# sloisel/MultiGridBarrier.jl

Measured on AMD Instinct MI355X. Metric: Newton iters/sec + wall-clock to converge, 2D P2 p-Laplace L=9, higher is better.
Workload: dtype f64

## Files before the change

multigridbarrier.jl_amd/csrc/api.cpp:

```cpp
#include <chrono>
#include <cmath>
#include <cstring>
#include <algorithm>
#include <limits>
#include <memory>
#include <string>

#include "closest.hpp"
#include "contour.hpp"
#include "faces.hpp"
#include "figure.hpp"
#include "interpolate.hpp"
#include "polyline.hpp"
#include "problem.hpp"
#include "quadrature.hpp"
#include "raycast.hpp"
#include "stream.hpp"
#include "surface.hpp"
#include "tubes.hpp"
#include "weld.hpp"

using namespace mgbhip;

mgbhip_problem* problem_create(mgbhip_ctx* ctx, const mgbhip_problem_desc* d, mgbhip_problem* share);
// ... 327 lines not shown
}

int mgbhip_set_hessian(mgbhip_problem* P, int32_t level, const double* values) {
    MGB_API_BEGIN_ON(P)
    check_level(P, level);
    MGB_REQUIRE(values, "null argument");
    P->ensure_plan(level);
    mgbhip::Level& L = P->levels[level];
    MGB_REQUIRE(L.Hval.n >= (size_t)L.nnz, "this level keeps no CSR value array");
    L.Hval.upload(values, (size_t)L.nnz, P->stream());
    MGB_HIP_CHECK(hipStreamSynchronize(P->stream()));
    L.H.set_from_outside();
    return MGBHIP_OK;
    MGB_API_END
}

int mgbhip_solve_newton(mgbhip_problem* P, int32_t level, const double* g, double* x, double* lambda2) {
    MGB_API_BEGIN_ON(P)
    check_level(P, level);
    MGB_REQUIRE(g && x, "null argument");
    hipStream_t st = P->stream();
    const size_t m = (size_t)P->levels[level].m;
    P->d_g.upload(g, m, st);
    P->factor(level, P->d_g.p);
    P->trisolve_carried(level, P->d_nv.p);
    int status = P->levels[level].solver.status(st);
    if (status != MGBHIP_OK && P->lu_fallback(level, P->d_g.p, P->d_nv.p)) status = MGBHIP_OK;
    P->d_nv.download(x, m, st);
    MGB_HIP_CHECK(hipStreamSynchronize(st));
    if (lambda2) {
        double acc = 0.0;
        for (size_t i = 0; i < m; ++i) acc += g[i] * x[i];
        *lambda2 = acc;
    }
    if (status != MGBHIP_OK) g_last_error = "Cholesky met a non-positive pivot";
    return status;
    MGB_API_END
}

int mgbhip_problem_set_sharding(mgbhip_problem* P, int32_t level, int64_t n_iface, const int32_t* iface_cols, const double* own_mask) {
    MGB_API_BEGIN_ON(P)
    check_level(P, level);
    mgbhip::Level& L = P->levels[level];
    MGB_REQUIRE(!L.solver.analyzed, "sharding must be set before the first solve of the level");
    MGB_REQUIRE(own_mask != nullptr && n_iface >= 0 && n_iface <= L.m && (n_iface == 0 || iface_cols), "bad sharding arguments");
    L.h_iface.assign(iface_cols, iface_cols + n_iface);
    for (int64_t i = 0; i < n_iface; ++i) {
// ... 8 lines not shown
    MGB_API_END
}

int mgbhip_problem_set_collective(mgbhip_problem* P, mgbhip_allreduce_fn fn, void* user, int32_t accepts_device_ptr) {
    MGB_API_BEGIN_ON(P)
    P->coll_fn = fn;
    P->coll_user = user;
    P->coll_device = accepts_device_ptr != 0;
    return MGBHIP_OK;
    MGB_API_END
}

int mgbhip_newton_direction(mgbhip_problem* P, int32_t level, const double* s, const double* c, const double* z0, double* x,
                            double* lambda2, int32_t* condensed) {
    MGB_API_BEGIN_ON(P)
    check_level(P, level);
    MGB_REQUIRE(s && c && z0 && x, "null argument");
    hipStream_t st = P->stream();
    const size_t m = (size_t)P->levels[level].m;
    stage_inputs(P, level, s, c, z0);
    P->eval_f1(level, P->d_x.p, P->d_z0.p, P->d_c.p, P->d_g.p);
    P->eval_f2(level, P->d_x.p, P->d_z0.p, P->d_c.p, false, P->d_g.p);
    if (condensed) *condensed = P->levels[level].H.condensed() ? 1 : 0;
    P->factor(level, P->d_g.p);
    P->trisolve_carried(level, P->d_nv.p);
    const int status = P->levels[level].solver.status(st);
    P->d_nv.download(x, m, st);
    if (lambda2) {
        std::vector<double> g(m);
        P->d_g.download(g.data(), m, st);
        MGB_HIP_CHECK(hipStreamSynchronize(st));
        double acc = 0.0;
        for (size_t i = 0; i < m; ++i) acc += g[i] * x[i];
        *lambda2 = acc;
    }
    MGB_HIP_CHECK(hipStreamSynchronize(st));
    if (status != MGBHIP_OK) g_last_error = "Cholesky met a non-positive pivot";
    return status;
    MGB_API_END
}

int mgbhip_trial_values(mgbhip_problem* P, int32_t level, const double* x, const double* dir, double step, const double* c,
                        const double* z0, double* y, double* g, double* xn, int32_t* moved, int32_t* finite, int32_t* path) {
    MGB_API_BEGIN_ON(P)
    check_level(P, level);
    MGB_REQUIRE(x && dir && c && z0 && y && g && xn && moved && finite && path, "null argument");
    MGB_REQUIRE(!P->sharded(), "trial_values: not for sharded problems");
// ... 1283 lines not shown
```

multigridbarrier.jl_amd/csrc/driver.cpp:

```cpp
#include <chrono>
#include <cstdio>
#include <cstdlib>
#include <cmath>
#include <cstring>
#include <functional>
#include <limits>

#include "problem.hpp"

using namespace mgbhip;

namespace {

constexpr double EPS = std::numeric_limits<double>::epsilon();

bool debug_on() {
    static const bool on = env_on("MGBHIP_DEBUG");
    return on;
}
#define DBG(...) do { if (debug_on()) { fprintf(stderr, __VA_ARGS__); } } while (0)

struct Stop {
    double lambda_tol;
    double theta;
// ... 172 lines not shown
        if (P->sharded()) { P->d_gpart.ensure((size_t)C.m); P->d_gnpart.ensure((size_t)C.m); }
        C.F1(P->d_x.p, P->d_g.p, P->d_gpart.p);
        gs = vec_stats(P, C.level, P->d_g.p, C.m);
    }
    double ymin = y;
    if (gs.bad != 0.0 || !std::isfinite(gs.sumsq)) throw InvalidArgument("newton: initial gradient has non-finite entries");
    double gnorm = std::sqrt(gs.sumsq);
    double gmin = gnorm;
    double incmin = INFINITY;
    int k = 0;
    bool converged = false;
    Level& L = P->levels[C.level];
    struct RobustReset {
        MfSolver& s;
        ~RobustReset() { s.robust = false; }
    } robust_reset{L.solver};
    while (k < maxit && !converged) {
        ++k;
        C.F2(P->d_x.p);
        auto t0 = std::chrono::steady_clock::now();
        int fstatus = MGBHIP_OK;
        int leaf_flag = 0;
        for (int attempt = 0; attempt < 2; ++attempt) {
            P->factor(C.level, C.rhs_of_g());
            P->trisolve_carried(C.level, P->d_nv.p);
            const double seq = P->next_seq();
            launch_dir_finish(P->d_nv.p, P->d_g.p, C.m, P->d_scratch.p, P->d_scal.p, L.solver.status_flags_rw(), P->pin.dev, st,
                              P->own_mask(C.level), seq);
            L.solver.flags_cleared();
            P->wait_results(seq);
            P->pin.i[1] = P->pin.d[5] != 0.0 ? 1 : 0;
            leaf_flag |= P->pin.d[6] != 0.0 ? 1 : 0;
            P->pin.i[2] = leaf_flag;
            fstatus = MfSolver::status_from(P->pin.i + 1, L.solver.factored_condensed);
            if (P->sharded()) {
                P->pin.d[5] = fstatus != MGBHIP_OK ? 1.0 : 0.0;
                P->allreduce_host(P->pin.d + 2, 4, 0);
                fstatus = P->pin.d[5] != 0.0 ? MGBHIP_ERR_NOT_SPD : MGBHIP_OK;
            }
            const bool at_floor = std::fabs(P->pin.d[4]) <= EPS * std::fmax(std::fabs(y), 1.0);
            const bool suspicious = fstatus != MGBHIP_OK || P->pin.d[3] != 0.0 || !std::isfinite(P->pin.d[2]) ||
                                    (!(P->pin.d[4] > 0) && !at_floor);
            if (!suspicious || attempt == 1 || !L.solver.has_inverse_path() || L.solver.robust) break;
            DBG("newton[lev %d] k=%d: direction rejected (status %d, lambda^2=%.3e): refactoring with the substitution kernels\n",
                C.level, k, fstatus, P->pin.d[4]);
            L.solver.robust = true;
            L.H.drop_factors();
// ... 288 lines not shown
```

multigridbarrier.jl_amd/csrc/kernels.hpp:

```cpp
#pragma once
#include "common.hpp"
#include "cone.hpp"
#include "elem_layout.hpp"
#include "panel_layout.hpp"

namespace mgbhip {

struct LeafDesc {
    int64_t F_off;
    int32_t interior;
    uint32_t packed;
};

struct ElemParams {
    int32_t p, nu, nD, nstage;
    int32_t ymask;
    int64_t N, n;
    const double* ops[MGBHIP_MAX_OPS];
    const double* stage_ptr[MGBHIP_MAX_OPS];
    int32_t D_state[MGBHIP_MAX_ND];
    int32_t D_op[MGBHIP_MAX_ND];
    int32_t D_stage[MGBHIP_MAX_ND];
    const double* w;
    const double* c;
// ... 60 lines not shown
void launch_restrict_trial(int64_t rows, const int32_t* ptr, const int32_t* col, const double* val, const double* ret, double* g,
                            double* scratch, const double* x, const double* nn, double s, double* xn, int32_t* moved, int32_t stamp,
                            hipStream_t st);
void launch_publish(const double* src, int n, double* host_block, int host_lo, double seq, hipStream_t st);
void launch_dir_finish(const double* v, const double* g, int64_t n, double* scratch, double* scal, int32_t* status2, double* host,
                       hipStream_t st, const double* mask = nullptr, double seq = 0.0);
void launch_trial_finish(const double* g, int64_t n, double* scratch, const double* f0_partials, int64_t f0_count, double* scal,
                         int32_t* moved, double* host, hipStream_t st, const double* mask = nullptr, double seq = 0.0,
                         bool partials_ready = false);
void launch_index_gather(const double* v, const int32_t* idx, int64_t cnt, double* out, hipStream_t st);
void launch_index_scatter(const double* in, const int32_t* idx, int64_t cnt, double* v, hipStream_t st);
int64_t reduce_scratch_doubles(int64_t n);

void launch_csr_matvec(int64_t rows, const int32_t* ptr, const int32_t* col, const double* val,
                       const double* x, double* y, bool add, bool long_rows, hipStream_t st);
int csr_chunks(int64_t max_row_len);
void launch_csr_matvec_chunked(int64_t rows, const int32_t* ptr, const int32_t* col, const double* val,
                               const double* x, double* y, double* scratch, int nchunk, hipStream_t st);
void launch_prolong(int64_t rows, const int32_t* ptr, const int32_t* col, const double* val, const double* s,
                    const double* z0, double* zfull, hipStream_t st);
void launch_step(const double* x, const double* n, double s, double* xn, int64_t len, int32_t* moved, int32_t stamp,
                 hipStream_t st);
void launch_scale_copy(const double* src, double alpha, double* dst, int64_t len, hipStream_t st);
void launch_border_tail(const double* g, double* tail, int64_t m, hipStream_t st);
void launch_axpy(double alpha, const double* x, double* y, int64_t len, hipStream_t st);
void launch_fill(double value, double* y, int64_t len, hipStream_t st);

void launch_gather_shared(int64_t nshared, const int32_t* sh_q, const int32_t* cptr, const int32_t* cidx, const double* slab,
                          double* out, hipStream_t st);
void launch_gather_assemble(int64_t nnz, const int32_t* cptr, const int32_t* cidx, const double* slab,
                            double* Hval, bool long_lists, hipStream_t st, int32_t chunk = 0, int32_t nchunk = 0,
                            double* part = nullptr, const int32_t* qmap = nullptr, int64_t nq = 0);

struct PanelParams {
    int32_t p, nu;
    int64_t N;
    const int32_t* ecol_ptr;
    const double* panels;
    const int32_t* eoff;
    const double* hel;
    double* slab;
    int32_t cmax;
    int32_t upper_only;
    const int32_t* spos;
};
bool launch_panel_project_mfma(const PanelParams& P, hipStream_t st);
void launch_invert_lists(const int32_t* cidx, int64_t total, int32_t* spos, hipStream_t st);
// ... 7 lines not shown
```

multigridbarrier.jl_amd/csrc/mf_launch_plan.hpp:

```cpp
#pragma once
#include <algorithm>
#include <cstdint>
#include <cstdlib>
#include <vector>

#include "host_util.hpp"
#include "mf_analysis.hpp"

namespace mgbhip {

struct MfLaunch {
    int32_t first, count;
    int32_t cls;
    int32_t max_m, max_k;
    int32_t max_child = 0;
    bool tiny = false;
    bool wave = false;
    bool inv = false;
    bool iface = false;
    int32_t grec_first = -1;
};

constexpr int BIG_INV_MAX_M = 7000;
constexpr int GATHER_MAX_CHILD = 8;
constexpr int BIG_DIAG0_MIN_COUNT = 24;

struct MfSwitches {
    bool no_geo;
    bool old_big;
    bool merge_groups;
    bool packed_leaves;
    bool wave_small;
    int64_t inv_min_n;
    int64_t wave_min_n;
    bool gather_lds_maps;
    int gather_ct;
    bool bwd_split;
    static MfSwitches from_env() {
        auto num = [](const char* name, long long dflt) { const char* e = getenv(name); return e ? atoll(e) : dflt; };
        return {env_on("MGBHIP_NO_GEO"), env_on("MGBHIP_OLD_BIG"), !env_on("MGBHIP_NO_MERGE_GROUPS"), !env_on("MGBHIP_NO_PACKED_LEAVES"),
                !env_on("MGBHIP_NO_WAVE_SMALL"), num("MGBHIP_INV_MIN_N", 1024), num("MGBHIP_WAVE_MIN_N", 0),
                env_on("MGBHIP_GATHER_LDS_MAPS"), (int)num("MGBHIP_GATHER_CT", 0), num("MGBHIP_BWD_SPLIT", 1) != 0};
    }
};

using LevelLaunches = std::vector<std::vector<MfLaunch>>;

inline MfLaunch launch_of_range(const MfPlan& plan, MfLaunch L, int32_t first, int32_t count) {
    L.first = first; L.count = count;
    L.max_m = 0; L.max_k = 0; L.max_child = 0;
    for (int32_t t = first; t < first + count; ++t) {
        L.max_m = std::max(L.max_m, plan.fronts[t].m);
        L.max_k = std::max(L.max_k, plan.fronts[t].k);
        L.max_child = std::max(L.max_child, plan.fronts[t].nchild);
    }
    return L;
}

inline void merge_straggler_groups(const MfPlan& plan, std::vector<MfLaunch>& G) {
    auto absorb = [&](size_t into, size_t from) {
        MfLaunch& A = G[into];
        const MfLaunch& B = G[from];
        A.first = B.first;
        A.count += B.count;
        A.max_k = std::max(A.max_k, B.max_k);
// ... 118 lines not shown
                    if (par >= 0 && on_big_path[par]) return false;
                    any = true;
                }
    return any;
}

enum MfAssembly : int32_t { MF_ASM_NONE = 0, MF_ASM_GATHER = 1, MF_ASM_COLS = 2 };
enum MfBlock0 : int32_t { MF_B0_NA = 0, MF_B0_GATHER = 1, MF_B0_DIAG0 = 2, MF_B0_STEP0 = 3 };
enum MfBackward : int32_t { MF_BWD_NA = 0, MF_BWD_K8 = 1, MF_BWD_K16 = 2, MF_BWD_GENERAL = 3 };

inline size_t big_gather_lds(const MfLaunch& L) { return (size_t)L.max_child * (size_t)L.max_m * sizeof(int32_t); }
inline MfAssembly big_assembly_kind(const MfLaunch& L) {
    if (L.cls) return MF_ASM_NONE;
    if (L.max_child < 1 || L.max_child > GATHER_MAX_CHILD || big_gather_lds(L) > 40 * 1024) return MF_ASM_COLS;
    return MF_ASM_GATHER;
}
inline MfBlock0 big_block0_kind(const MfLaunch& L, bool inv) {
    if (L.cls || !inv) return MF_B0_NA;
    if (!L.iface && big_assembly_kind(L) == MF_ASM_GATHER) return MF_B0_GATHER;
    return (L.iface || L.count >= BIG_DIAG0_MIN_COUNT) ? MF_B0_DIAG0 : MF_B0_STEP0;
}
inline int backward_small_kmax(const MfLaunch& L) { return L.max_k <= 8 ? 8 : (L.max_k <= 16 ? 16 : 0); }

constexpr int GATHER_MIN_WGS = 768;
inline int big_gather_ct(const MfLaunch& L, int forced) {
    if (forced == 8 || forced == 16 || forced == 32) return forced;
    int ct = 8;
    while (ct < 32 && (int64_t)L.count * ((L.max_m + 2 * ct - 1) / (2 * ct)) >= GATHER_MIN_WGS) ct *= 2;
    return ct;
}

constexpr int BWD_SPLIT_MAX = 16;
constexpr int BWD_SPLIT_CUS = 256;
constexpr int BWD_SPLIT_COLS = 64;
constexpr int BWD_THIN_BOUNDARY = 8;
inline int bwd_inv_split(int32_t count, int32_t max_k, int32_t max_m) {
    if (count < 1 || max_m - max_k <= BWD_THIN_BOUNDARY) return 1;
    return std::max(1, std::min({BWD_SPLIT_MAX, BWD_SPLIT_CUS / count, (max_k + BWD_SPLIT_COLS - 1) / BWD_SPLIT_COLS}));
}
inline int32_t bwd_split_stride(int32_t max_k) { return (max_k + 1) & ~1; }
inline void bwd_split_scratch(const LevelLaunches& solves, int64_t out[2]) {
    out[0] = out[1] = 0;
    for (auto& lev : solves)
        for (auto& L : lev) {
            if (L.count == 0 || L.cls || !L.inv || bwd_inv_split(L.count, L.max_k, L.max_m) == 1) continue;
            out[0] = std::max<int64_t>(out[0], L.count);
// ... 61 lines not shown
```

multigridbarrier.jl_amd/csrc/mf_numeric.hip:

```cpp
#include <hip/hip_runtime.h>

#include <cstdio>

#include <algorithm>
#include <cstdlib>

#include "../../include/mgbhip.h"
#include "mf_solver.hpp"
#include "mf_device.hpp"
#include "mf_small.hpp"
#include "mf_big_subst.hpp"
#include "mf_big_inv.hpp"

namespace mgbhip {

namespace {

int32_t query_lds_cap() {
    if (hipFuncSetAttribute((const void*)mf_factor_small<8, true>, hipFuncAttributeMaxDynamicSharedMemorySize,
                            (int)factor_small_lds(128)) == hipSuccess)
        return 128;
    (void)hipGetLastError();
    return 88;
}
// ... 148 lines not shown
            if (!L.cls) max_big = std::max(max_big, L.count);
        }
    d_dscr.alloc((size_t)max_big * 2 * NB * NB);
    {
        int64_t need[2] = {0, 0};
        if (sw.bwd_split) bwd_split_scratch(level_solves, need);
        if (need[0] == 0) { d_bwd_g.release(); d_bwd_cnt.release(); }
        else {
            d_bwd_g.alloc((size_t)need[1]);
            d_bwd_cnt.alloc((size_t)need[0]);
            d_bwd_cnt.zero(st);
        }
    }

    std::vector<int64_t> ug_ptr, ug_src;
    build_gather_lists(plan, on_big_path, fd, ug_ptr, ug_src);
    leaf_packed = sw.packed_leaves && pack_leaf_fronts(plan, level_launches, on_big_path, fd);
    d_ug_ptr.upload(ug_ptr, st);
    d_ug_src.upload(ug_src, st);
    std::vector<GatherRec> grec;
    std::vector<int32_t> gmap;
    if (!sw.gather_lds_maps) build_gather_maps(plan, level_launches, grec, gmap);
    gather_ct = sw.gather_ct;
    if (grec.empty()) { d_grec.release(); d_gmap.release(); }
    else { d_grec.upload(grec, st); d_gmap.upload(gmap, st); }
    d_fronts.upload(fd, st);
    h_fronts = fd;
    h_a_dst = remap_a_dst(plan, level_launches);
    d_a_dst.upload(h_a_dst, st);
    if (debug_level() >= 2) dump_plan(plan, level_launches);
    analyzed = true;
    MGB_HIP_CHECK(hipStreamSynchronize(st));
}

void MfSolver::set_direct_map(const int32_t* value_map, int64_t nnz, int64_t tail_base, hipStream_t st) {
    std::vector<int32_t> as(plan.a_src.size());
    for (size_t t = 0; t < as.size(); ++t) {
        const int64_t src = plan.a_src[t];
        const int64_t v = src < nnz ? (int64_t)value_map[src] : tail_base + (src - nnz);
        MGB_REQUIRE(v < (int64_t)INT32_MAX, "direct value index exceeds 32 bits");
        as[t] = (int32_t)v;
    }
    d_a_src_direct.upload(as, st);
    MGB_HIP_CHECK(hipStreamSynchronize(st));
}

void MfSolver::factor(const double* d_values, hipStream_t st, StageTimers* timers, bool direct, bool condensed) {
    MGB_REQUIRE(!direct || d_a_src_direct.n > 0, "MfSolver::factor: no direct value map");
    MGB_REQUIRE(!condensed || (direct && condensed_ok), "MfSolver::factor: condensed leaves are not enabled");
    MGB_REQUIRE(analyzed, "MfSolver::factor before analyze");
    const FactorArgs a{condensed ? d_fronts_c.p : d_fronts.p, d_children.p, d_rel.p,
                       condensed ? d_a_src_c.p : (direct ? d_a_src_direct.p : d_a_src.p), condensed ? d_a_dst_c.p : d_a_dst.p,
                       condensed ? d_a_colptr_c.p : d_a_colptr.p, d_values, d_arena.p, d_dscr.p, d_dvec.p, d_status.p, st,
                       d_grec.n ? d_grec.p : nullptr, d_gmap.p, gather_ct};
    if (timers) timers->begin("factor");
    factored_inv = !robust;
    if (!status_zero) MGB_HIP_CHECK(hipMemsetAsync(d_status.p, 0, sizeof(int32_t), st));
    status_zero = false;
    factored_condensed = condensed;
    int lvno = -1;
    for (auto& lev : level_launches) {
        LevelScope lvscope(timers, "fac", ++lvno);
        for (auto& L : lev) {
            if (L.count == 0) continue;
            if (condensed && lvno == 0) continue;
            if (L.tiny) launch_factor_tiny(a, L);
            else if (L.wave && L.cls <= 32) launch_factor_wave<32>(a, L);
            else if (L.wave) launch_factor_wave<48>(a, L);
            else if (L.cls) launch_factor_small(a, L);
            else {
                const bool inv = L.inv && !robust;
                const MfBlock0 b0 = big_block0_kind(L, inv);
                MGB_REQUIRE(!L.iface || (bool)iface_reduce, "MfSolver: interface front without a reduction hook");
                launch_big_assemble(a, L, b0 == MF_B0_GATHER);
                if (L.iface) {
                    const Front& fi = plan.fronts[L.first];
                    const int64_t tri = (int64_t)fi.m * (fi.m + 1) / 2;
                    d_ifpack.ensure((size_t)tri);
                    launch_tri_pack(fi.m, d_arena.p + fi.F_off, d_ifpack.p, false, st);
                    iface_reduce(d_ifpack.p, tri);
                    launch_tri_pack(fi.m, d_arena.p + fi.F_off, d_ifpack.p, true, st);
                }
                if (inv) {
                    if (b0 == MF_B0_DIAG0) launch_big_diag0(a, L, L.count);
                    launch_inv_steps(a, L, L.count, b0 == MF_B0_STEP0);
                } else
                    launch_subst_steps(a, L, L.count);
            }
        }
    }
    MGB_HIP_CHECK(hipGetLastError());
    if (timers) timers->end();
}

void MfSolver::solve(const double* d_b, double* d_x, hipStream_t st, StageTimers* timers) {
    MGB_REQUIRE(analyzed, "MfSolver::solve before analyze");
    if (timers) timers->begin("trisolve");
    const size_t n = (size_t)plan.n;
    MGB_HIP_CHECK(hipMemcpyAsync(d_bx.p, d_b, n * sizeof(double), hipMemcpyDeviceToDevice, st));
    MGB_HIP_CHECK(hipMemsetAsync(d_bx.p + n, 0, sizeof(double), st));
    forward_pass(d_bx.p, st, timers);
    backward_pass(d_xx.p, st, timers);
    MGB_HIP_CHECK(hipMemcpyAsync(d_x, d_xx.p, n * sizeof(double), hipMemcpyDeviceToDevice, st));
    MGB_HIP_CHECK(hipGetLastError());
    if (timers) timers->end();
}

void MfSolver::solve_border(double* d_x_np1, hipStream_t st, StageTimers* timers) {
    MGB_REQUIRE(analyzed, "MfSolver::solve_border before analyze");
    if (timers) timers->begin("trisolve");
    const size_t n = (size_t)plan.n;
    if (!y_zero) {
        MGB_HIP_CHECK(hipMemsetAsync(d_y.p, 0, n * sizeof(double), st));
        y_zero = true;
    }
    if (!y_border_one) {
        MGB_HIP_CHECK(hipMemcpyAsync(d_y.p + n, d_one.p, sizeof(double), hipMemcpyDeviceToDevice, st));
        y_border_one = true;
    }
    backward_pass(d_x_np1, st, timers);
    MGB_HIP_CHECK(hipGetLastError());
    if (timers) timers->end();
}

void MfSolver::forward_pass(const double* d_b, hipStream_t st, StageTimers* timers) {
    y_border_one = false;
    y_zero = false;
    const SolveArgs a = solve_args(d_b, nullptr, st);
    int lvno = -1;
    for (auto& lev : level_solves) {
        LevelScope lvscope(timers, "fwd", ++lvno);
        for (auto& L : lev) {
            if (L.count == 0) continue;
            if (L.tiny) launch_forward_tiny(a, L);
            else if (L.cls) launch_forward_small(a, L);
            else if (L.inv && factored_inv) launch_fwd_inv(a, L);
            else if (L.max_m <= BIG1_MAX_M) launch_fwd_big1(a, L);
            else launch_fwd_big_steps(a, L);
        }
    }
}

void MfSolver::backward_pass(double* d_x, hipStream_t st, StageTimers* timers) {
    const SolveArgs a = solve_args(nullptr, d_x, st);
    for (int32_t l = (int32_t)level_solves.size() - 1; l >= 0; --l) {
        LevelScope lvscope(timers, "bwd", l);
        for (auto it = level_solves[l].rbegin(); it != level_solves[l].rend(); ++it) {
            const MfLaunch& L = *it;
            if (L.count == 0) continue;
            if (L.tiny) launch_backward_tiny(a, L);
            else if (L.cls) launch_backward_small(a, L);
            else if (L.inv && factored_inv) launch_bwd_inv(a, L);
            else if (L.max_m <= BIG1_MAX_M) launch_bwd_big1(a, L);
            else launch_bwd_big_steps(a, L);
        }
    }
}

#ifdef MGB_STEP_PROBE
void mf_debug_probe(long long* out64) {
    (void)hipMemcpyFromSymbol(out64, HIP_SYMBOL(g_probe), 64 * sizeof(long long));
    long long init[64];
    for (int i = 0; i < 64; ++i) init[i] = 0;
    init[56] = 0x7fffffffffffffffll;
    (void)hipMemcpyToSymbol(HIP_SYMBOL(g_probe), init, sizeof(init));
}
#endif

// ... 114 lines not shown
```

multigridbarrier.jl_amd/csrc/mf_small.hpp:

```cpp
#pragma once
#include "mf_device.hpp"

namespace mgbhip {
namespace {

template <int NBT, bool PACKED>
__global__ void mf_factor_small(const FrontDev* __restrict__ fr, int32_t first,
                                const int32_t* __restrict__ children, const int32_t* __restrict__ rel,
                                const int32_t* __restrict__ a_src, const int32_t* __restrict__ a_dst,
                                const double* __restrict__ Hval, double* __restrict__ arena,
                                int32_t* __restrict__ status) {
    extern __shared__ double W[];
    const FrontDev F = fr[first + blockIdx.x];
    double* Fg = arena + F.F_off;
    const int m = F.m, k = F.k;
    const int tid = threadIdx.x, nt = blockDim.x;
    const int tx = tid % TX, ty = tid / TX, TYn = nt / TX;
    const int mm = PACKED ? m * (m + 1) / 2 : m * m;
    auto co = [m](int c) { return PACKED ? c * (m - 1) - c * (c - 1) / 2 : c * m; };
    double* S = W + mm;

    SP(0);
    int a_d0 = -1;
    double a_v0 = 0.0;
// ... 18 lines not shown
    __shared__ int64_t cU[CHILD_CHUNK];
    __shared__ int64_t cR[CHILD_CHUNK];
    __shared__ int32_t cM[CHILD_CHUNK], cB[CHILD_CHUNK];
    __shared__ int32_t crl[128];
    __shared__ double prinv[32];
    for (int cbase = 0; cbase < F.nchild; cbase += CHILD_CHUNK) {
        const int nc = min(CHILD_CHUNK, F.nchild - cbase);
        __syncthreads();
        if (tid < nc) {
            if (cbase == 0) {
                cU[tid] = pU; cR[tid] = pR; cM[tid] = pM; cB[tid] = pB;
            } else {
                const FrontDev C = fr[children[F.child_off + cbase + tid]];
                int64_t u_; int32_t m_;
                child_update_desc(C, u_, m_);
                cU[tid] = u_;
                cR[tid] = C.rel_off;
                cM[tid] = m_;
                cB[tid] = C.m - C.k;
            }
        }
        __syncthreads();
        for (int c0 = 0; c0 < nc; c0 += 4) {
            if (nt == 256 && (c0 & 15) == 0) {
                const int ng = min(16, nc - c0);
                bool small16 = true;
                for (int u = 0; u < ng; ++u) small16 = small16 && cB[c0 + u] * cB[c0 + u] <= 64;
                if (small16) {
                    const int w = tid >> 6, e = tid & 63;
                    int dst[4];
                    double val[4];
#pragma unroll
                    for (int u = 0; u < 4; ++u) {
                        dst[u] = -1;
                        val[u] = 0.0;
                        const int c = c0 + 4 * w + u;
                        if (4 * w + u < ng) {
                            const int b = cB[c];
                            if (e < b * b) {
                                const int j = e / b, r = e - j * b;
                                if (r >= j) {
                                    const int32_t* rl = rel + cR[c];
                                    dst[u] = rl[r] + co(rl[j]);
                                    val[u] = arena[child_entry(cU[c], cM[c], j, r)];
                                }
                            }
                        }
// ... 519 lines not shown
    const FrontDev F = fr[first + (on ? fi : 0)];
    const int m = F.m, k = on ? F.k : 0;
    const int32_t* idx = front_idx + F.idx_off;
    const double* Fm = arena + F.F_off;
    const bool row = on && r < m;
    const int myidx = row ? idx[r] : 0;
    double t = row ? ((r < k) ? y[myidx] : x[myidx]) : 0.0;
    double l[16];
#pragma unroll
    for (int j = 0; j < 16; ++j) l[j] = (row && j < k && r > j) ? Fm[tiny_entry(F, r, j)] : 0.0;
    int kmax = k;
    kmax = max(kmax, __shfl_xor(kmax, 16, 64));
    kmax = max(kmax, __shfl_xor(kmax, 32, 64));
#pragma unroll
    for (int j = 15; j >= 0; --j) {
        if (j >= kmax) continue;
        double s = l[j] * t;
        s = row16_sum_f64(s);
        if (r == j && j < k) t -= s;
    }
    if (row && r < k) x[myidx] = t;
}

inline size_t factor_small_lds(int cls) {
    return (size_t)((cls >= 88 ? cls * (cls + 1) / 2 : cls * cls) + 8 * cls) * sizeof(double);
}
inline void launch_factor_small(const FactorArgs& a, const MfLaunch& L) {
    const int threads = L.cls <= 16 ? 64 : (L.cls <= 32 ? 128 : 256);
    if (L.cls >= 88)
        hipLaunchKernelGGL((mf_factor_small<8, true>), dim3(L.count), dim3(threads), factor_small_lds(L.cls), a.st, a.fr, L.first,
                           a.children, a.rel, a.a_src, a.a_dst, a.values, a.arena, a.status);
    else
        hipLaunchKernelGGL((mf_factor_small<8, false>), dim3(L.count), dim3(threads), factor_small_lds(L.cls), a.st, a.fr, L.first,
                           a.children, a.rel, a.a_src, a.a_dst, a.values, a.arena, a.status);
}

template <int MW>
inline size_t factor_wave_lds() {
    return (size_t)4 * (MW * (MW + 1) / 2) * sizeof(double) + 4 * 64 * (sizeof(int64_t) + sizeof(int32_t));
}
template <int MW>
inline void launch_factor_wave(const FactorArgs& a, const MfLaunch& L) {
    hipLaunchKernelGGL(mf_factor_wave<MW>, dim3((L.count + 3) / 4), dim3(256), factor_wave_lds<MW>(), a.st, a.fr, L.first, L.count,
                       a.children, a.rel, a.a_src, a.a_dst, a.values, a.arena, a.status);
}

inline void launch_factor_tiny(const FactorArgs& a, const MfLaunch& L) {
    hipLaunchKernelGGL(mf_factor_tiny, dim3((L.count + 15) / 16), dim3(256), 0, a.st, a.fr, L.first, L.count, a.a_src, a.a_dst,
                       a.values, a.arena, a.status);
}

// ... 30 lines not shown
```

multigridbarrier.jl_amd/csrc/mf_solver.hpp:

```cpp
#pragma once
#include <functional>

#include "common.hpp"
#include "mf_analysis.hpp"
#include "mf_launch_plan.hpp"
#include "kernels.hpp"

namespace mgbhip {

struct FrontDev {
    int32_t k, m, nchild, a_cnt;
    int64_t F_off, idx_off, u_off, child_off, rel_off, a_off, acol_off;
    int64_t ug_off;
    int32_t packed;
    int32_t pad_;
};

struct FactorArgs {
    const FrontDev* fr;
    const int32_t *children, *rel, *a_src, *a_dst, *a_colptr;
    const double* values;
    double *arena, *dscr, *dvec;
    int32_t* status;
    hipStream_t st;
    const GatherRec* grec;
    const int32_t* gmap;
    int gather_ct;
};
struct SolveArgs {
    const FrontDev* fr;
    const int32_t *front_idx, *children, *rel;
    const int64_t *ug_ptr, *ug_src;
    const double *arena, *dvec;
    const double* b;
    double *y, *x, *uvec, *tbig, *tsol;
    hipStream_t st;
    double* bwd_g;
    uint32_t* bwd_cnt;
};

class MfSolver {
   public:
    MfPlan plan;
    void analyze(int64_t n, const int32_t* rowptr, const int32_t* colidx, hipStream_t st,
                 const double* coords = nullptr, int dim = 0, bool protect_peeled = false,
                 const int32_t* top = nullptr, int64_t ntop = 0);
    std::function<void(double*, int64_t)> iface_reduce;
    void factor(const double* d_values, hipStream_t st, StageTimers* timers, bool direct = false, bool condensed = false);
    bool enable_condensed(int64_t N, int P, const int32_t* ucol, int64_t slack0, int64_t nnz, int64_t tail_base, hipStream_t st);
    bool condensed_ready() const { return condensed_ok; }
    bool leaves_packed() const { return leaf_packed; }
    const LeafDesc* leaf_desc() const { return d_leaf_desc.p; }
    double* arena() { return d_arena.p; }
    int32_t* leaf_status() { return d_status.p + 1; }
    const int32_t* status_flags() const { return d_status.p; }
    int32_t* status_flags_rw() { return d_status.p; }
    void flags_cleared() { status_zero = true; leaf_zero = true; }
    bool leaf_flag_zero() const { return leaf_zero; }
    void leaf_flag_used() { leaf_zero = false; }
    void set_direct_map(const int32_t* value_map, int64_t nnz, int64_t tail_base, hipStream_t st);
    bool has_direct_map() const { return d_a_src_direct.n > 0; }
    void solve(const double* d_b, double* d_x, hipStream_t st, StageTimers* timers);
    void solve_border(double* d_x_np1, hipStream_t st, StageTimers* timers);
    void chain_stats(double* out8) const;
    int64_t launches(int32_t* out, int64_t cap) const;
    int status(hipStream_t st);
    void status_async(int32_t* h_dst, hipStream_t st) const;
    static int status_from(const int32_t* flags2, bool with_leaves) {
        return (flags2[0] || (with_leaves && flags2[1])) ? MGBHIP_ERR_NOT_SPD : MGBHIP_OK;
    }
    bool factored_condensed = false;
    bool analyzed = false;
    bool robust = false;
    bool has_inverse_path() const { return uses_inv; }
    bool factored_inv = false;

   private:
    void upload_plan(hipStream_t st);
    SolveArgs solve_args(const double* d_b, double* d_x, hipStream_t st) const {
        return {d_fronts.p, d_front_idx.p, d_children.p, d_rel.p, d_ug_ptr.p, d_ug_src.p, d_arena.p, d_dvec.p, d_b, d_y.p, d_x,
                d_uvec.p, d_tbig.p, d_tsol.p, st, d_bwd_g.p, d_bwd_cnt.n ? d_bwd_cnt.p : nullptr};
    }
    void forward_pass(const double* d_b_np1, hipStream_t st, StageTimers* timers);
    void backward_pass(double* d_x_np1, hipStream_t st, StageTimers* timers);
    DevBuf<double> d_bx, d_xx, d_one;
    DevBuf<FrontDev> d_fronts;
    DevBuf<int32_t> d_front_idx, d_children, d_rel, d_a_src, d_a_src_direct, d_a_dst, d_a_colptr;
    DevBuf<GatherRec> d_grec;
    DevBuf<int32_t> d_gmap;
    DevBuf<int64_t> d_ug_ptr, d_ug_src;
    DevBuf<double> d_arena, d_uvec, d_y, d_tbig, d_tsol, d_dscr, d_dvec;
    DevBuf<double> d_ifpack;
    DevBuf<int32_t> d_status;
    DevBuf<double> d_bwd_g;
    DevBuf<uint32_t> d_bwd_cnt;
    bool condensed_ok = false;
    bool leaf_packed = false;
    std::vector<FrontDev> h_fronts;
    std::vector<int32_t> h_a_dst;
    DevBuf<FrontDev> d_fronts_c;
    DevBuf<int32_t> d_a_src_c, d_a_dst_c, d_a_colptr_c;
    DevBuf<LeafDesc> d_leaf_desc;
    std::vector<std::vector<MfLaunch>> level_launches;
    std::vector<std::vector<MfLaunch>> level_solves;
    int gather_ct = 0;
    int32_t lds_cap = 88;
    bool uses_inv = false;
    bool y_border_one = false;
    bool y_zero = false;
    bool status_zero = false, leaf_zero = false;
};

}
```

multigridbarrier.jl_amd/csrc/problem.cpp:

```cpp
#include "problem.hpp"
#include "assembly_plan.hpp"
#include "plan_device.hpp"
#include "dense.hpp"

#include <algorithm>
#include <cmath>
#include <cstdio>
#include <atomic>
#include <exception>
#include <cstdlib>
#include <string>
#include <thread>
#include <cstring>
#include <numeric>

using namespace mgbhip;



static void upload_csr(const mgbhip_csr& R, Level& L, hipStream_t st) {
    MGB_REQUIRE(R.rows >= 0 && R.cols >= 0 && R.rowptr && (R.rowptr[R.rows] == 0 || (R.colidx && R.values)),
                "bad prolongation CSR");
    MGB_REQUIRE(R.rows < INT32_MAX && R.cols < INT32_MAX, "prolongation too large for 32-bit indices");
    L.rows = R.rows;
// ... 789 lines not shown
        }
    }
}

void mgbhip_problem::ensure_direct(int level) {
    Level& L = levels[level];
    if (!(L.selection && L.direct) || dense || !L.solver.analyzed) return;
    hipStream_t st = stream();
    const bool dbg2 = debug_level() >= 2;
    if (!L.solver.has_direct_map()) {
        const Stopwatch sw;
        L.solver.set_direct_map(L.h_vmap.data(), L.nnz, hel_cap + L.nshared, st);
        std::vector<int32_t>().swap(L.h_vmap);
        if (dbg2) fprintf(stderr, "[mgbhip] direct value map level %d: %.2f s\n", level, sw.seconds());
    }
    if (!L.condense_tried) {
        const Stopwatch sw;
        L.condense_tried = true;
        L.condense = try_enable_condensed(level);
        if (dbg2) fprintf(stderr, "[mgbhip] condensed-leaf set-up level %d: %.2f s\n", level, sw.seconds());
    }
}

void mgbhip_problem::factor(int level, const double* rhs) {
    Level& L = levels[level];
    const FactorPlan plan = L.H.about_to_factor(hel_owner, level, rhs);
    hipStream_t st = stream();
    ensure_analysis(level);
    if (plan.slab()) {
        ensure_direct(level);
        launch_border_tail(rhs, d_hel.p + hel_cap + L.nshared, L.m, st);
        L.solver.factor(d_hel.p, st, &ctx->timers, true, plan.condensed());
    } else {
        if (plan.write == HTail::Rhs) {
            launch_border_tail(rhs, L.Hval.p + L.nnz, L.m, st);
        } else if (plan.write == HTail::Identity) {
            MGB_HIP_CHECK(hipMemsetAsync(L.Hval.p + L.nnz, 0, sizeof(double) * (size_t)L.m, st));
            launch_fill(1.0, L.Hval.p + L.nnz + L.m, 1, st);
        }
        L.solver.factor(L.Hval.p, st, &ctx->timers);
    }
    L.H.factors_ready(plan);
    cnt.factor++;
}

bool mgbhip_problem::lu_fallback(int level, const double* d_g, double* d_xout) {
    Level& L = levels[level];
    static const bool off = env_on("MGBHIP_NO_LU_FALLBACK");
    if (off || sharded() || !L.H.in_csr() || L.m < 1 || L.m > DENSE_LU_MAX_M || L.Hval.n < (size_t)L.nnz || !L.Hptr.p || !L.Hcol.p)
        return false;
    hipStream_t st = stream();
    d_lu.ensure((size_t)L.m * (size_t)L.m);
    d_lustat.ensure(1);
    d_lustat.zero(st, 1);
    launch_dense_lu_solve((int)L.m, L.Hptr.p, L.Hcol.p, L.Hval.p, d_lu.p, d_g, d_xout, d_lustat.p, st);
    int32_t bad = 1;
    d_lustat.download(&bad, 1, st);
    MGB_HIP_CHECK(hipStreamSynchronize(st));
    if (bad == 0) ++lu_fallbacks;
    return bad == 0;
}

void mgbhip_problem::trisolve(int level, const double* d_g, double* d_xout) {
// ... 11 lines not shown
```

multigridbarrier.jl_amd/csrc/problem.hpp:

```cpp
#pragma once
#include <mutex>
#include <memory>
#include <string>
#include <vector>

#include "../../include/mgbhip.h"
#include "common.hpp"
#include "hessian_state.hpp"
#include "kernels.hpp"
#include "mf_solver.hpp"

struct mgbhip_ctx {
    int device = 0;
    hipStream_t stream = nullptr;
    bool own_stream = false;
    mgbhip::StageTimers timers;
    mgbhip::DevBuf<double> vscratch, vscal;
};

struct mgbhip_vec {
    mgbhip_ctx* ctx = nullptr;
    mgbhip::DevBuf<double> buf;
    int64_t len = 0;
};
// ... 115 lines not shown
    hipStream_t stream() const { return ctx->stream; }
    void ensure_plan(int level);
    void ensure_analysis(int level);
    void ensure_direct(int level);
    void prepare_all();
    double next_seq() { return ++result_seq; }
    void wait_results(double seq);
    bool can_fuse_step(int level) const;
    void read_scalars(int lo, int n);
    double result_seq = 0.0;
    std::mutex shared_mutex;
    bool prepared = false;
    void ensure_plan_dense(int level);
    double eval_f0(int level, const double* d_s, const double* d_zz, const double* d_cc);
    void eval_f0_launch(int level, const double* d_s, const double* d_zz, const double* d_cc);
    void eval_f1(int level, const double* d_s, const double* d_zz, const double* d_cc, double* d_gout, double* d_part = nullptr);
    bool eval_f01_launch(int level, const double* d_s, const double* d_zz, const double* d_cc, double* d_gout, double* d_part = nullptr,
                         bool defer_f0_sum = false, const mgbhip::TrialPoint* trial = nullptr, const mgbhip::TrialRestrict* fuse = nullptr);
    void eval_f2(int level, const double* d_s, const double* d_zz, const double* d_cc, bool materialize = true,
                 const double* rhs = nullptr);
    bool try_enable_condensed(int level);
    int64_t hel_cap = 0;
    mgbhip::SlabOwner hel_owner;
    void factor(int level, const double* rhs = nullptr);
    void trisolve(int level, const double* d_g, double* d_xout);
    void trisolve_carried(int level, double* d_xout_np1);
    bool lu_fallback(int level, const double* d_g, double* d_xout);
    mgbhip::DevBuf<double> d_lu;
    mgbhip::DevBuf<int32_t> d_lustat;
    int64_t lu_fallbacks = 0;
};
```

multigridbarrier.jl_amd/csrc/vector_kernels.hpp:

```cpp
#pragma once
#include "reduce_kernels.hpp"

namespace mgbhip {

namespace {


template <bool ADD>
__global__ __launch_bounds__(256) void csr_matvec_row_kernel(int64_t rows, const int32_t* __restrict__ ptr,
                                                             const int32_t* __restrict__ col,
                                                             const double* __restrict__ val,
                                                             const double* __restrict__ x, double* __restrict__ y) {
    const int64_t i = (int64_t)blockIdx.x * 256 + threadIdx.x;
    if (i >= rows) return;
    double s = 0.0;
    for (int32_t q = ptr[i]; q < ptr[i + 1]; ++q) s += val[q] * x[col[q]];
    y[i] = ADD ? y[i] + s : s;
}

template <bool ADD>
__global__ __launch_bounds__(256) void csr_matvec_wave_kernel(int64_t rows, const int32_t* __restrict__ ptr,
                                                              const int32_t* __restrict__ col,
                                                              const double* __restrict__ val,
                                                              const double* __restrict__ x, double* __restrict__ y) {
// ... 65 lines not shown
                                                   int32_t* __restrict__ moved, int32_t stamp) {
    const int64_t i = (int64_t)blockIdx.x * 256 + threadIdx.x;
    bool m = false;
    if (i < len) {
        const double xi = x[i];
        const double v = __builtin_fma(-s, nn[i], xi);
        xn[i] = v;
        m = (v != xi);
    }
    __shared__ int any_moved;
    if (threadIdx.x == 0) any_moved = 0;
    __syncthreads();
    if (m) any_moved = 1;
    __syncthreads();
    if (threadIdx.x == 0 && any_moved) *moved = stamp;
}

__global__ __launch_bounds__(256) void scale_copy_kernel(const double* __restrict__ src, double alpha,
                                                         double* __restrict__ dst, int64_t len) {
    const int64_t i = (int64_t)blockIdx.x * 256 + threadIdx.x;
    if (i < len) dst[i] = alpha * src[i];
}

__global__ __launch_bounds__(256) void border_tail_kernel(const double* __restrict__ g, double* __restrict__ tail, int64_t m) {
    const int64_t i = (int64_t)blockIdx.x * 256 + threadIdx.x;
    if (i < m) tail[i] = -1.0 * g[i];
    else if (i == m) tail[i] = -1.0;
}

__global__ __launch_bounds__(256) void axpy_kernel(double alpha, const double* __restrict__ x,
                                                   double* __restrict__ y, int64_t len) {
    const int64_t i = (int64_t)blockIdx.x * 256 + threadIdx.x;
    if (i < len) y[i] += alpha * x[i];
}

__global__ __launch_bounds__(256) void fill_kernel(double value, double* __restrict__ y, int64_t len) {
    const int64_t i = (int64_t)blockIdx.x * 256 + threadIdx.x;
    if (i < len) y[i] = value;
}

}

__global__ __launch_bounds__(256) void index_gather_kernel(const double* __restrict__ v, const int32_t* __restrict__ idx,
                                                           int64_t cnt, double* __restrict__ out) {
    const int64_t i = (int64_t)blockIdx.x * 256 + threadIdx.x;
    if (i < cnt) out[i] = v[idx[i]];
}
__global__ __launch_bounds__(256) void index_scatter_kernel(const double* __restrict__ in, const int32_t* __restrict__ idx,
                                                            int64_t cnt, double* __restrict__ v) {
    const int64_t i = (int64_t)blockIdx.x * 256 + threadIdx.x;
// ... 38 lines not shown
}

void launch_prolong(int64_t rows, const int32_t* ptr, const int32_t* col, const double* val, const double* s,
                    const double* z0, double* zfull, hipStream_t st) {
    if (rows == 0) return;
    hipLaunchKernelGGL(prolong_kernel, dim3((unsigned)((rows + 255) / 256)), dim3(256), 0, st, rows, ptr, col, val, s,
                       z0, zfull);
    MGB_HIP_CHECK(hipGetLastError());
}

void launch_step(const double* x, const double* n, double s, double* xn, int64_t len, int32_t* moved, int32_t stamp,
                 hipStream_t st) {
    if (len == 0) return;
    hipLaunchKernelGGL(step_kernel, dim3((unsigned)((len + 255) / 256)), dim3(256), 0, st, x, n, s, xn, len, moved, stamp);
    MGB_HIP_CHECK(hipGetLastError());
}

void launch_scale_copy(const double* src, double alpha, double* dst, int64_t len, hipStream_t st) {
    if (len == 0) return;
    hipLaunchKernelGGL(scale_copy_kernel, dim3((unsigned)((len + 255) / 256)), dim3(256), 0, st, src, alpha, dst, len);
    MGB_HIP_CHECK(hipGetLastError());
}

void launch_border_tail(const double* g, double* tail, int64_t m, hipStream_t st) {
    hipLaunchKernelGGL(border_tail_kernel, dim3((unsigned)((m + 1 + 255) / 256)), dim3(256), 0, st, g, tail, m);
    MGB_HIP_CHECK(hipGetLastError());
}

void launch_axpy(double alpha, const double* x, double* y, int64_t len, hipStream_t st) {
    if (len == 0) return;
    hipLaunchKernelGGL(axpy_kernel, dim3((unsigned)((len + 255) / 256)), dim3(256), 0, st, alpha, x, y, len);
    MGB_HIP_CHECK(hipGetLastError());
}

void launch_fill(double value, double* y, int64_t len, hipStream_t st) {
    if (len == 0) return;
    hipLaunchKernelGGL(fill_kernel, dim3((unsigned)((len + 255) / 256)), dim3(256), 0, st, value, y, len);
    MGB_HIP_CHECK(hipGetLastError());
}

}
```

Baseline: 702.9.

## Skip solitary border front in factor and solve, adapt small-factor thread count

When the bordered Newton system's last elimination level holds only the border column (a 1x1 front), the factorization now stops before it. The border tail kernel writes the known unit entry of the carried solution directly, and the backward pass skips that level, saving kernel launches on each Newton step. Separately, the small-front factor kernel now picks 256, 512 or 1024 threads from LDS fit and front count per compute unit to raise occupancy. Both rely on new invariants: solve() is forbidden on carried factors, and the border pivot check is no longer done, which might affect status detection.

```diff
diff --git a/multigridbarrier.jl_amd/csrc/api.cpp b/multigridbarrier.jl_amd/csrc/api.cpp
--- a/multigridbarrier.jl_amd/csrc/api.cpp
+++ b/multigridbarrier.jl_amd/csrc/api.cpp
@@ -373,7 +373,7 @@
     hipStream_t st = P->stream();
     const size_t m = (size_t)P->levels[level].m;
     P->d_g.upload(g, m, st);
-    P->factor(level, P->d_g.p);
+    P->factor(level, P->d_g.p, P->d_nv.p);
     P->trisolve_carried(level, P->d_nv.p);
     int status = P->levels[level].solver.status(st);
     if (status != MGBHIP_OK && P->lu_fallback(level, P->d_g.p, P->d_nv.p)) status = MGBHIP_OK;
@@ -428,7 +428,7 @@
     P->eval_f1(level, P->d_x.p, P->d_z0.p, P->d_c.p, P->d_g.p);
     P->eval_f2(level, P->d_x.p, P->d_z0.p, P->d_c.p, false, P->d_g.p);
     if (condensed) *condensed = P->levels[level].H.condensed() ? 1 : 0;
-    P->factor(level, P->d_g.p);
+    P->factor(level, P->d_g.p, P->d_nv.p);
     P->trisolve_carried(level, P->d_nv.p);
     const int status = P->levels[level].solver.status(st);
     P->d_nv.download(x, m, st);
diff --git a/multigridbarrier.jl_amd/csrc/driver.cpp b/multigridbarrier.jl_amd/csrc/driver.cpp
--- a/multigridbarrier.jl_amd/csrc/driver.cpp
+++ b/multigridbarrier.jl_amd/csrc/driver.cpp
@@ -218,7 +218,7 @@
         int fstatus = MGBHIP_OK;
         int leaf_flag = 0;
         for (int attempt = 0; attempt < 2; ++attempt) {
-            P->factor(C.level, C.rhs_of_g());
+            P->factor(C.level, C.rhs_of_g(), P->d_nv.p);
             P->trisolve_carried(C.level, P->d_nv.p);
             const double seq = P->next_seq();
             launch_dir_finish(P->d_nv.p, P->d_g.p, C.m, P->d_scratch.p, P->d_scal.p, L.solver.status_flags_rw(), P->pin.dev, st,
diff --git a/multigridbarrier.jl_amd/csrc/kernels.hpp b/multigridbarrier.jl_amd/csrc/kernels.hpp
--- a/multigridbarrier.jl_amd/csrc/kernels.hpp
+++ b/multigridbarrier.jl_amd/csrc/kernels.hpp
@@ -106,7 +106,7 @@
 void launch_step(const double* x, const double* n, double s, double* xn, int64_t len, int32_t* moved, int32_t stamp,
                  hipStream_t st);
 void launch_scale_copy(const double* src, double alpha, double* dst, int64_t len, hipStream_t st);
-void launch_border_tail(const double* g, double* tail, int64_t m, hipStream_t st);
+void launch_border_tail(const double* g, double* tail, int64_t m, hipStream_t st, double* x_one = nullptr);
 void launch_axpy(double alpha, const double* x, double* y, int64_t len, hipStream_t st);
 void launch_fill(double value, double* y, int64_t len, hipStream_t st);
 
diff --git a/multigridbarrier.jl_amd/csrc/mf_launch_plan.hpp b/multigridbarrier.jl_amd/csrc/mf_launch_plan.hpp
--- a/multigridbarrier.jl_amd/csrc/mf_launch_plan.hpp
+++ b/multigridbarrier.jl_amd/csrc/mf_launch_plan.hpp
@@ -36,11 +36,14 @@
     bool gather_lds_maps;
     int gather_ct;
     bool bwd_split;
+    int small_threads;
+    bool border_launches;
     static MfSwitches from_env() {
         auto num = [](const char* name, long long dflt) { const char* e = getenv(name); return e ? atoll(e) : dflt; };
         return {env_on("MGBHIP_NO_GEO"), env_on("MGBHIP_OLD_BIG"), !env_on("MGBHIP_NO_MERGE_GROUPS"), !env_on("MGBHIP_NO_PACKED_LEAVES"),
                 !env_on("MGBHIP_NO_WAVE_SMALL"), num("MGBHIP_INV_MIN_N", 1024), num("MGBHIP_WAVE_MIN_N", 0),
-                env_on("MGBHIP_GATHER_LDS_MAPS"), (int)num("MGBHIP_GATHER_CT", 0), num("MGBHIP_BWD_SPLIT", 1) != 0};
+                env_on("MGBHIP_GATHER_LDS_MAPS"), (int)num("MGBHIP_GATHER_CT", 0), num("MGBHIP_BWD_SPLIT", 1) != 0,
+                (int)num("MGBHIP_SMALL_THREADS", 0), env_on("MGBHIP_BORDER_LAUNCHES")};
     }
 };
 
@@ -205,6 +208,25 @@
 }
 inline int backward_small_kmax(const MfLaunch& L) { return L.max_k <= 8 ? 8 : (L.max_k <= 16 ? 16 : 0); }
 
+inline size_t factor_small_lds(int cls) {
+    return (size_t)((cls >= 88 ? cls * (cls + 1) / 2 : cls * cls) + 8 * cls) * sizeof(double);
+}
+constexpr int SMALL_STATIC_LDS = 2112;
+constexpr int CU_LDS_BYTES = 160 * 1024;
+constexpr int SMALL_FILL_WAVES = 24;
+inline int factor_small_threads(const MfLaunch& L, int compute_units, int forced = 0) {
+    if (L.cls <= 16) return 64;
+    if (L.cls <= 32) return 128;
+    if (forced == 256 || forced == 512 || forced == 1024) return forced;
+    const int64_t cu = std::max(compute_units, 1);
+    const int64_t fit = std::max<int64_t>(1, CU_LDS_BYTES / (int64_t)(factor_small_lds(L.cls) + SMALL_STATIC_LDS));
+    const int64_t per_cu = std::min(fit, ((int64_t)L.count + cu - 1) / cu);
+    int threads = 256;
+    while (threads < 1024 && per_cu * (2 * threads / 64) <= SMALL_FILL_WAVES) threads *= 2;
+    return threads;
+}
+static_assert(16 - 1 <= 64 && 32 - 1 <= 128 && 128 - 1 <= 256, "mf_factor_small solves one panel row per thread");
+
 constexpr int GATHER_MIN_WGS = 768;
 inline int big_gather_ct(const MfLaunch& L, int forced) {
     if (forced == 8 || forced == 16 || forced == 32) return forced;
diff --git a/multigridbarrier.jl_amd/csrc/mf_numeric.hip b/multigridbarrier.jl_amd/csrc/mf_numeric.hip
--- a/multigridbarrier.jl_amd/csrc/mf_numeric.hip
+++ b/multigridbarrier.jl_amd/csrc/mf_numeric.hip
@@ -194,6 +194,24 @@
     std::vector<int32_t> gmap;
     if (!sw.gather_lds_maps) build_gather_maps(plan, level_launches, grec, gmap);
     gather_ct = sw.gather_ct;
+    small_threads = sw.small_threads;
+    {
+        int dev = 0, cus = 0;
+        MGB_HIP_CHECK(hipGetDevice(&dev));
+        MGB_HIP_CHECK(hipDeviceGetAttribute(&cus, hipDeviceAttributeMultiprocessorCount, dev));
+        compute_units = std::max(cus, 1);
+    }
+    border_launches = sw.border_launches;
+    {
+        const int32_t nlev = (int32_t)plan.level_ptr.size() - 1;
+        border_alone = false;
+        if (plan.border && nlev >= 2 && plan.level_ptr[nlev] - plan.level_ptr[nlev - 1] == 1) {
+            const Front& f = plan.fronts[plan.level_ptr[nlev - 1]];
+            border_alone = f.m == 1 && f.k == 1 && plan.front_idx[f.idx_off] == (int32_t)plan.n;
+        }
+    }
+    border_skipped = false;
+    carried_x = nullptr;
     if (grec.empty()) { d_grec.release(); d_gmap.release(); }
     else { d_grec.upload(grec, st); d_gmap.upload(gmap, st); }
     d_fronts.upload(fd, st);
@@ -217,21 +235,29 @@
     MGB_HIP_CHECK(hipStreamSynchronize(st));
 }
 
-void MfSolver::factor(const double* d_values, hipStream_t st, StageTimers* timers, bool direct, bool condensed) {
+bool MfSolver::skips_border() const {
+    return analyzed && border_alone && !border_launches && !robust && plan.iface_front < 0;
+}
+
+void MfSolver::factor(const double* d_values, hipStream_t st, StageTimers* timers, bool direct, bool condensed, double* carried_x_np1) {
     MGB_REQUIRE(!direct || d_a_src_direct.n > 0, "MfSolver::factor: no direct value map");
     MGB_REQUIRE(!condensed || (direct && condensed_ok), "MfSolver::factor: condensed leaves are not enabled");
     MGB_REQUIRE(analyzed, "MfSolver::factor before analyze");
     const FactorArgs a{condensed ? d_fronts_c.p : d_fronts.p, d_children.p, d_rel.p,
                        condensed ? d_a_src_c.p : (direct ? d_a_src_direct.p : d_a_src.p), condensed ? d_a_dst_c.p : d_a_dst.p,
                        condensed ? d_a_colptr_c.p : d_a_colptr.p, d_values, d_arena.p, d_dscr.p, d_dvec.p, d_status.p, st,
-                       d_grec.n ? d_grec.p : nullptr, d_gmap.p, gather_ct};
+                       d_grec.n ? d_grec.p : nullptr, d_gmap.p, gather_ct, small_threads, compute_units};
     if (timers) timers->begin("factor");
     factored_inv = !robust;
+    border_skipped = carried_x_np1 != nullptr && skips_border();
+    carried_x = border_skipped ? carried_x_np1 : nullptr;
+    const int border_level = (int)level_launches.size() - 1;
     if (!status_zero) MGB_HIP_CHECK(hipMemsetAsync(d_status.p, 0, sizeof(int32_t), st));
     status_zero = false;
     factored_condensed = condensed;
     int lvno = -1;
     for (auto& lev : level_launches) {
+        if (border_skipped && lvno + 1 == border_level) break;
         LevelScope lvscope(timers, "fac", ++lvno);
         for (auto& L : lev) {
             if (L.count == 0) continue;
@@ -267,6 +293,7 @@
 
 void MfSolver::solve(const double* d_b, double* d_x, hipStream_t st, StageTimers* timers) {
     MGB_REQUIRE(analyzed, "MfSolver::solve before analyze");
+    MGB_REQUIRE(!border_skipped, "MfSolver::solve on factors that carry a Newton right-hand side");
     if (timers) timers->begin("trisolve");
     const size_t n = (size_t)plan.n;
     MGB_HIP_CHECK(hipMemcpyAsync(d_bx.p, d_b, n * sizeof(double), hipMemcpyDeviceToDevice, st));
@@ -290,7 +317,9 @@
         MGB_HIP_CHECK(hipMemcpyAsync(d_y.p + n, d_one.p, sizeof(double), hipMemcpyDeviceToDevice, st));
         y_border_one = true;
     }
-    backward_pass(d_x_np1, st, timers);
+    if (border_skipped && d_x_np1 != carried_x)
+        MGB_HIP_CHECK(hipMemcpyAsync(d_x_np1 + n, d_one.p, sizeof(double), hipMemcpyDeviceToDevice, st));
+    backward_pass(d_x_np1, st, timers, border_skipped);
     MGB_HIP_CHECK(hipGetLastError());
     if (timers) timers->end();
 }
@@ -313,9 +342,9 @@
     }
 }
 
-void MfSolver::backward_pass(double* d_x, hipStream_t st, StageTimers* timers) {
+void MfSolver::backward_pass(double* d_x, hipStream_t st, StageTimers* timers, bool without_border) {
     const SolveArgs a = solve_args(nullptr, d_x, st);
-    for (int32_t l = (int32_t)level_solves.size() - 1; l >= 0; --l) {
+    for (int32_t l = (int32_t)level_solves.size() - (without_border ? 2 : 1); l >= 0; --l) {
         LevelScope lvscope(timers, "bwd", l);
         for (auto it = level_solves[l].rbegin(); it != level_solves[l].rend(); ++it) {
             const MfLaunch& L = *it;
diff --git a/multigridbarrier.jl_amd/csrc/mf_small.hpp b/multigridbarrier.jl_amd/csrc/mf_small.hpp
--- a/multigridbarrier.jl_amd/csrc/mf_small.hpp
+++ b/multigridbarrier.jl_amd/csrc/mf_small.hpp
@@ -64,7 +64,7 @@
         }
         __syncthreads();
         for (int c0 = 0; c0 < nc; c0 += 4) {
-            if (nt == 256 && (c0 & 15) == 0) {
+            if (nt >= 256 && (c0 & 15) == 0) {
                 const int ng = min(16, nc - c0);
                 bool small16 = true;
                 for (int u = 0; u < ng; ++u) small16 = small16 && cB[c0 + u] * cB[c0 + u] <= 64;
@@ -630,11 +630,9 @@
     if (row && r < k) x[myidx] = t;
 }
 
-inline size_t factor_small_lds(int cls) {
-    return (size_t)((cls >= 88 ? cls * (cls + 1) / 2 : cls * cls) + 8 * cls) * sizeof(double);
-}
 inline void launch_factor_small(const FactorArgs& a, const MfLaunch& L) {
-    const int threads = L.cls <= 16 ? 64 : (L.cls <= 32 ? 128 : 256);
+    const int threads = factor_small_threads(L, a.compute_units, a.small_threads);
+    MGB_REQUIRE(threads >= L.max_m - 1, "mf_factor_small: fewer threads than panel rows");
     if (L.cls >= 88)
         hipLaunchKernelGGL((mf_factor_small<8, true>), dim3(L.count), dim3(threads), factor_small_lds(L.cls), a.st, a.fr, L.first,
                            a.children, a.rel, a.a_src, a.a_dst, a.values, a.arena, a.status);
diff --git a/multigridbarrier.jl_amd/csrc/mf_solver.hpp b/multigridbarrier.jl_amd/csrc/mf_solver.hpp
--- a/multigridbarrier.jl_amd/csrc/mf_solver.hpp
+++ b/multigridbarrier.jl_amd/csrc/mf_solver.hpp
@@ -26,6 +26,8 @@
     const GatherRec* grec;
     const int32_t* gmap;
     int gather_ct;
+    int small_threads;
+    int compute_units;
 };
 struct SolveArgs {
     const FrontDev* fr;
@@ -46,7 +48,9 @@
                  const double* coords = nullptr, int dim = 0, bool protect_peeled = false,
                  const int32_t* top = nullptr, int64_t ntop = 0);
     std::function<void(double*, int64_t)> iface_reduce;
-    void factor(const double* d_values, hipStream_t st, StageTimers* timers, bool direct = false, bool condensed = false);
+    void factor(const double* d_values, hipStream_t st, StageTimers* timers, bool direct = false, bool condensed = false,
+                double* carried_x = nullptr);
+    bool skips_border() const;
     bool enable_condensed(int64_t N, int P, const int32_t* ucol, int64_t slack0, int64_t nnz, int64_t tail_base, hipStream_t st);
     bool condensed_ready() const { return condensed_ok; }
     bool leaves_packed() const { return leaf_packed; }
@@ -82,7 +86,7 @@
                 d_uvec.p, d_tbig.p, d_tsol.p, st, d_bwd_g.p, d_bwd_cnt.n ? d_bwd_cnt.p : nullptr};
     }
     void forward_pass(const double* d_b_np1, hipStream_t st, StageTimers* timers);
-    void backward_pass(double* d_x_np1, hipStream_t st, StageTimers* timers);
+    void backward_pass(double* d_x_np1, hipStream_t st, StageTimers* timers, bool without_border = false);
     DevBuf<double> d_bx, d_xx, d_one;
     DevBuf<FrontDev> d_fronts;
     DevBuf<int32_t> d_front_idx, d_children, d_rel, d_a_src, d_a_src_direct, d_a_dst, d_a_colptr;
@@ -104,6 +108,12 @@
     std::vector<std::vector<MfLaunch>> level_launches;
     std::vector<std::vector<MfLaunch>> level_solves;
     int gather_ct = 0;
+    int small_threads = 0;
+    int compute_units = 1;
+    bool border_launches = false;
+    bool border_alone = false;
+    bool border_skipped = false;
+    const double* carried_x = nullptr;
     int32_t lds_cap = 88;
     bool uses_inv = false;
     bool y_border_one = false;
diff --git a/multigridbarrier.jl_amd/csrc/problem.cpp b/multigridbarrier.jl_amd/csrc/problem.cpp
--- a/multigridbarrier.jl_amd/csrc/problem.cpp
+++ b/multigridbarrier.jl_amd/csrc/problem.cpp
@@ -835,23 +835,25 @@
     }
 }
 
-void mgbhip_problem::factor(int level, const double* rhs) {
+void mgbhip_problem::factor(int level, const double* rhs, double* carried_out) {
     Level& L = levels[level];
     const FactorPlan plan = L.H.about_to_factor(hel_owner, level, rhs);
     hipStream_t st = stream();
     ensure_analysis(level);
+    double* const carried_x = (plan.write == HTail::Rhs && carried_out && !sharded() && L.solver.skips_border()) ? carried_out : nullptr;
+    double* const x_one = carried_x ? carried_x + L.m : nullptr;
     if (plan.slab()) {
         ensure_direct(level);
-        launch_border_tail(rhs, d_hel.p + hel_cap + L.nshared, L.m, st);
-        L.solver.factor(d_hel.p, st, &ctx->timers, true, plan.condensed());
+        launch_border_tail(rhs, d_hel.p + hel_cap + L.nshared, L.m, st, x_one);
+        L.solver.factor(d_hel.p, st, &ctx->timers, true, plan.condensed(), carried_x);
     } else {
         if (plan.write == HTail::Rhs) {
-            launch_border_tail(rhs, L.Hval.p + L.nnz, L.m, st);
+            launch_border_tail(rhs, L.Hval.p + L.nnz, L.m, st, x_one);
         } else if (plan.write == HTail::Identity) {
             MGB_HIP_CHECK(hipMemsetAsync(L.Hval.p + L.nnz, 0, sizeof(double) * (size_t)L.m, st));
             launch_fill(1.0, L.Hval.p + L.nnz + L.m, 1, st);
         }
-        L.solver.factor(L.Hval.p, st, &ctx->timers);
+        L.solver.factor(L.Hval.p, st, &ctx->timers, false, false, carried_x);
     }
     L.H.factors_ready(plan);
     cnt.factor++;
diff --git a/multigridbarrier.jl_amd/csrc/problem.hpp b/multigridbarrier.jl_amd/csrc/problem.hpp
--- a/multigridbarrier.jl_amd/csrc/problem.hpp
+++ b/multigridbarrier.jl_amd/csrc/problem.hpp
@@ -161,7 +161,7 @@
     bool try_enable_condensed(int level);
     int64_t hel_cap = 0;
     mgbhip::SlabOwner hel_owner;
-    void factor(int level, const double* rhs = nullptr);
+    void factor(int level, const double* rhs = nullptr, double* carried_out = nullptr);
     void trisolve(int level, const double* d_g, double* d_xout);
     void trisolve_carried(int level, double* d_xout_np1);
     bool lu_fallback(int level, const double* d_g, double* d_xout);
diff --git a/multigridbarrier.jl_amd/csrc/vector_kernels.hpp b/multigridbarrier.jl_amd/csrc/vector_kernels.hpp
--- a/multigridbarrier.jl_amd/csrc/vector_kernels.hpp
+++ b/multigridbarrier.jl_amd/csrc/vector_kernels.hpp
@@ -111,10 +111,14 @@
     if (i < len) dst[i] = alpha * src[i];
 }
 
-__global__ __launch_bounds__(256) void border_tail_kernel(const double* __restrict__ g, double* __restrict__ tail, int64_t m) {
+__global__ __launch_bounds__(256) void border_tail_kernel(const double* __restrict__ g, double* __restrict__ tail, int64_t m,
+                                                          double* __restrict__ x_one) {
     const int64_t i = (int64_t)blockIdx.x * 256 + threadIdx.x;
     if (i < m) tail[i] = -1.0 * g[i];
-    else if (i == m) tail[i] = -1.0;
+    else if (i == m) {
+        tail[i] = -1.0;
+        if (x_one) *x_one = 1.0;
+    }
 }
 
 __global__ __launch_bounds__(256) void axpy_kernel(double alpha, const double* __restrict__ x,
@@ -199,8 +203,8 @@
     MGB_HIP_CHECK(hipGetLastError());
 }
 
-void launch_border_tail(const double* g, double* tail, int64_t m, hipStream_t st) {
-    hipLaunchKernelGGL(border_tail_kernel, dim3((unsigned)((m + 1 + 255) / 256)), dim3(256), 0, st, g, tail, m);
+void launch_border_tail(const double* g, double* tail, int64_t m, hipStream_t st, double* x_one) {
+    hipLaunchKernelGGL(border_tail_kernel, dim3((unsigned)((m + 1 + 255) / 256)), dim3(256), 0, st, g, tail, m, x_one);
     MGB_HIP_CHECK(hipGetLastError());
 }
 
```

After: 716.7, median of 6. 2.0% higher.
